# bcgsc/ntLink

Hardware: AMD Instinct MI355X
Metric: read Gbases/s mapped (ntLink pair, paf=True) (higher is better)
Workload: dtype u64

## Files before the change

include/ntlink_amd.h:

```cpp
#ifndef NTLINK_AMD_H
#define NTLINK_AMD_H

#include <stdint.h>

#ifdef __cplusplus
extern "C" {
#endif

#define NTL_OK 0
#define NTL_EINVAL (-1)
#define NTL_EDEVICE (-2)
#define NTL_ENOMEM (-3)
#define NTL_EINTERNAL (-4)
#define NTL_ERANGE (-5)
#define NTL_EIO (-6)

typedef struct ntl_ctx ntl_ctx;
typedef struct ntl_batch ntl_batch;
typedef struct ntl_sketch ntl_sketch;
typedef struct ntl_index ntl_index;
typedef struct ntl_mapres ntl_mapres;


int ntl_ctx_create(int device, ntl_ctx **out);
// ... 2 lines not shown
const char *ntl_ctx_device_name(const ntl_ctx *ctx);
int ntl_ctx_sync(ntl_ctx *ctx);
int ntl_ctx_pipelined(const ntl_ctx *ctx);
int ntl_ctx_set_pipeline(ntl_ctx *ctx, int on);
int ntl_ctx_side_stream(const ntl_ctx *ctx);

int ntl_prof_enable(ntl_ctx *ctx, int on);
int ntl_prof_reset(ntl_ctx *ctx);
int ntl_prof_get(ntl_ctx *ctx, const char *name, double *total_ms, uint64_t *launches);


int ntl_batch_create(ntl_ctx *ctx, const char *seqs, const uint64_t *offsets, uint64_t nseq,
                     ntl_batch **out);
void ntl_batch_destroy(ntl_batch *b);
uint64_t ntl_packed_words(uint64_t bases);
int ntl_batch_create_packed(ntl_ctx *ctx, const uint32_t *packed, const uint64_t *offsets, uint64_t nseq,
                            const uint32_t *seq_run_first, const uint32_t *run_start, const uint32_t *run_len, uint64_t nruns,
                            ntl_batch **out);
int ntl_batch_create_packed_at(ntl_ctx *ctx, const uint32_t *packed, uint64_t span_positions, const uint64_t *positions,
                               const uint32_t *lengths, uint64_t nseq, const uint32_t *seq_run_first, const uint32_t *run_start,
                               const uint32_t *run_len, uint64_t nruns, ntl_batch **out);
uint64_t ntl_batch_nseq(const ntl_batch *b);
uint64_t ntl_batch_bases(const ntl_batch *b);

int ntl_host_alloc(ntl_ctx *ctx, uint64_t bytes, void **out);
void ntl_host_free(ntl_ctx *ctx, void *p);


int ntl_synth_genome(ntl_ctx *ctx, uint64_t seed, const uint32_t *len, uint64_t nseq, ntl_batch **out);
int ntl_synth_slices(ntl_ctx *ctx, const ntl_batch *src, uint64_t seed, uint64_t n, const uint32_t *src_seq,
                     const uint32_t *src_start, const uint32_t *out_len, const uint8_t *reverse,
                     double sub, double ins, double del, ntl_batch **out);
int ntl_batch_download(const ntl_batch *b, char *seqs, uint64_t *offsets);


int ntl_batch_mask(ntl_ctx *ctx, const ntl_batch *src, uint64_t n, const uint32_t *src_seq, const uint32_t *keep_lo,
                   const uint32_t *keep_hi, ntl_batch **out);
int ntl_batch_download_n(const ntl_batch *b, char *seqs, uint64_t *offsets);


typedef struct ntl_ascii ntl_ascii;
typedef struct ntl_stitched ntl_stitched;
typedef struct { uint32_t store, rec, lo, hi, flags; } ntl_stitch_seg;
#define NTL_STITCH_FILL 0xFFFFFFFFu
#define NTL_STITCH_REVCOMP 1u
#define NTL_STITCH_LOWER 2u
// ... 243 lines not shown
```

ntlink_amd/capi.py:

```python
import ctypes as C
import threading
import weakref
import os

import numpy as np
from time import perf_counter as _now

_HERE = os.path.dirname(os.path.abspath(__file__))
DEFAULT_LIB = os.path.join(_HERE, "libntlink_hip.so")

SYMBOLS = [
    "ntl_ctx_create", "ntl_ctx_destroy", "ntl_last_error", "ntl_ctx_device_name", "ntl_ctx_sync", "ntl_ctx_pipelined", "ntl_ctx_set_pipeline", "ntl_ctx_side_stream",
    "ntl_prof_enable", "ntl_prof_reset", "ntl_prof_get",
    "ntl_batch_create", "ntl_batch_create_packed", "ntl_batch_create_packed_at", "ntl_packed_words", "ntl_batch_destroy", "ntl_batch_nseq", "ntl_batch_bases", "ntl_host_alloc", "ntl_host_free",
    "ntl_synth_genome", "ntl_synth_slices", "ntl_batch_download", "ntl_batch_mask", "ntl_batch_download_n",
    "ntl_ascii_create", "ntl_ascii_destroy", "ntl_ascii_nrec", "ntl_ascii_bytes", "ntl_stitch", "ntl_stitched_bytes", "ntl_stitched_copy", "ntl_stitched_destroy",
    "ntl_stitched_base_counts",
    "ntl_sketch_run", "ntl_sketch_run_indexed", "ntl_sketch_run_for_map", "ntl_sketch_has_records", "ntl_sketch_destroy", "ntl_sketch_nseq", "ntl_sketch_count", "ntl_sketch_download",
    "ntl_sketch_strips", "ntl_sketch_redo_strips", "ntl_sketch_fallback_strips", "ntl_sketch_from_lists", "ntl_sketch_plan", "ntl_sketch_wait", "ntl_mapres_wait",
    "ntl_sketch_from_host", "ntl_overlap_filter", "ntl_overlap_cuts", "ntl_path_chains",
    "ntl_index_build", "ntl_index_destroy", "ntl_index_size",
    "ntl_map_run", "ntl_mapres_destroy", "ntl_mapres_n_mappings", "ntl_mapres_n_hits", "ntl_mapres_n_pafs",
    "ntl_mapres_n_index_hits", "ntl_mapres_download", "ntl_mapres_from_host", "ntl_mapres_liftover", "ntl_map_run_grouped", "ntl_mapres_grouped_info", "ntl_mapres_gap_cuts",
    "ntl_fastx_open", "ntl_fastx_open_range", "ntl_fastx_range", "ntl_fastx_close", "ntl_fastx_error", "ntl_fastx_next", "ntl_fastx_sizes", "ntl_fastx_copy", "ntl_fastx_copy_packed", "ntl_fastx_runs", "ntl_fastx_next_span", "ntl_fastx_parse_span", "ntl_fastx_copy_span", "ntl_fastx_seqs", "ntl_fastx_offsets",
    "ntl_fastx_names", "ntl_fastx_name_offsets", "ntl_write_indexlr", "ntl_write_verbose", "ntl_write_paf",
    "ntl_tsv_open", "ntl_tsv_close", "ntl_tsv_error", "ntl_tsv_next", "ntl_tsv_sizes", "ntl_tsv_copy",
    "ntl_vmap_open", "ntl_vmap_close", "ntl_vmap_error", "ntl_vmap_next", "ntl_vmap_sizes", "ntl_vmap_copy",
    "ntl_gap_pair_table", "ntl_gap_select", "ntl_gap_cands_count", "ntl_gap_cands_copy", "ntl_gap_cands_destroy",
    "ntl_tally_create", "ntl_tally_destroy", "ntl_tally_add", "ntl_tally_npairs", "ntl_tally_ngaps", "ntl_tally_export", "ntl_tally_merge",
    "ntl_liftover",
    "ntl_names_create", "ntl_names_destroy", "ntl_mapres_format", "ntl_text_sizes", "ntl_text_download", "ntl_text_destroy", "ntl_write_blob",
    "ntl_tally_add_ends", "ntl_tally_write", "ntl_io_errno",
    "ntl_pairtab_create", "ntl_pairtab_destroy", "ntl_mapres_pairs", "ntl_pairs_count", "ntl_pairs_download", "ntl_pairs_destroy", "ntl_tally_add_pairs",
]

MAPPING_DT = np.dtype([("read", "<u4"), ("ctg", "<u4"), ("n_hits", "<u4"), ("pad", "<u4"), ("hit_off", "<u8")])
HIT_DT = np.dtype([("ctg_pos", "<u4"), ("read_pos", "<u4"), ("ctg_strand", "u1"), ("read_strand", "u1"),
# ... 74 lines not shown
    L.ntl_ctx_sync.argtypes = [vp]
    L.ntl_ctx_pipelined.argtypes = [vp]
    L.ntl_ctx_set_pipeline.argtypes = [vp, C.c_int]
    L.ntl_ctx_side_stream.argtypes = [vp]
    L.ntl_sketch_wait.argtypes = [vp]
    L.ntl_mapres_wait.argtypes = [vp]
    L.ntl_prof_enable.argtypes = [vp, C.c_int]
    L.ntl_prof_reset.argtypes = [vp]
    L.ntl_prof_get.argtypes = [vp, C.c_char_p, C.POINTER(C.c_double), u64p]
    L.ntl_batch_create.argtypes = [vp, vp, u64p, C.c_uint64, C.POINTER(vp)]
    L.ntl_batch_create_packed.argtypes = [vp, vp, u64p, C.c_uint64, vp, vp, vp, C.c_uint64, C.POINTER(vp)]
    L.ntl_batch_create_packed_at.argtypes = [vp, vp, C.c_uint64, vp, vp, C.c_uint64, vp, vp, vp, C.c_uint64, C.POINTER(vp)]
    L.ntl_fastx_next_span.argtypes = [vp, C.c_uint64, u64p, u64p]
    L.ntl_fastx_parse_span.argtypes = [vp, vp, u64p, u64p, u64p, u64p]
    L.ntl_fastx_copy_span.argtypes = [vp, vp, vp, vp, vp, vp, vp, vp, u64p]
    L.ntl_packed_words.argtypes = [C.c_uint64]
    L.ntl_packed_words.restype = C.c_uint64
    L.ntl_batch_destroy.argtypes = [vp]
    L.ntl_batch_destroy.restype = None
    L.ntl_batch_nseq.argtypes = [vp]
    L.ntl_batch_nseq.restype = C.c_uint64
    L.ntl_batch_bases.argtypes = [vp]
    L.ntl_batch_bases.restype = C.c_uint64
    L.ntl_synth_genome.argtypes = [vp, C.c_uint64, u32p, C.c_uint64, C.POINTER(vp)]
    L.ntl_synth_slices.argtypes = [vp, vp, C.c_uint64, C.c_uint64, u32p, u32p, u32p, u8p, C.c_double, C.c_double, C.c_double,
                                   C.POINTER(vp)]
    L.ntl_batch_download.argtypes = [vp, vp, u64p]
    L.ntl_batch_mask.argtypes = [vp, vp, C.c_uint64, u32p, u32p, u32p, C.POINTER(vp)]
    L.ntl_batch_download_n.argtypes = [vp, vp, u64p]
    L.ntl_ascii_create.argtypes = [vp, vp, u64p, C.c_uint64, C.POINTER(vp)]
    L.ntl_ascii_destroy.argtypes = [vp]
    L.ntl_ascii_destroy.restype = None
    for nm in ("ntl_ascii_nrec", "ntl_ascii_bytes", "ntl_stitched_bytes"):
        getattr(L, nm).argtypes = [vp]
        getattr(L, nm).restype = C.c_uint64
    L.ntl_stitch.argtypes = [vp, C.POINTER(vp), C.c_uint32, vp, C.c_uint64, C.POINTER(vp)]
    L.ntl_stitched_copy.argtypes = [vp, C.c_uint64, C.c_uint64, vp]
    L.ntl_stitched_destroy.argtypes = [vp]
    L.ntl_stitched_destroy.restype = None
    L.ntl_stitched_base_counts.argtypes = [vp, u64p, C.c_uint64, u64p]
    L.ntl_sketch_run.argtypes = [vp, vp, C.c_int, C.c_int, C.POINTER(vp)]
    L.ntl_sketch_run_indexed.argtypes = [vp, vp, C.c_int, C.c_int, vp, C.POINTER(vp)]
    L.ntl_sketch_run_for_map.argtypes = [vp, vp, C.c_int, C.c_int, vp, C.POINTER(vp)]
    L.ntl_sketch_has_records.argtypes = [vp]
    L.ntl_sketch_destroy.argtypes = [vp]
    L.ntl_sketch_destroy.restype = None
# ... 137 lines not shown
        try:
            self.close()
        except Exception:
            pass

    def __enter__(self):
        return self

    def __exit__(self, *a):
        self.close()


class Batch(_Handle):
    _destroy = "ntl_batch_destroy"

    @property
    def nseq(self):
        return int(self.dev.L.ntl_batch_nseq(self.ptr))

    @property
    def bases(self):
        return int(self.dev.L.ntl_batch_bases(self.ptr))

    def download(self):
        buf = np.empty(max(self.bases, 1), np.uint8)
        off = np.zeros(self.nseq + 1, np.uint64)
        self.dev._chk(self.dev.L.ntl_batch_download(self.ptr, buf.ctypes.data, _ptr(off, C.c_uint64)))
        return buf[:self.bases], off

    def download_n(self):
        off = np.zeros(self.nseq + 1, np.uint64)
        buf = np.empty(max(self.bases, 1), np.uint8)
        self.dev._chk(self.dev.L.ntl_batch_download_n(self.ptr, buf.ctypes.data, _ptr(off, C.c_uint64)))
        return buf[:int(off[-1])], off


class Ascii(_Handle):
    _destroy = "ntl_ascii_destroy"

    @property
    def nrec(self):
        return int(self.dev.L.ntl_ascii_nrec(self.ptr))

    @property
    def nbytes(self):
        return int(self.dev.L.ntl_ascii_bytes(self.ptr))
# ... 537 lines not shown
```

ntlink_amd/csrc/ntl_hip.hip:

```cpp
#include <hip/hip_runtime.h>
#include <stdint.h>
#include <stdio.h>
#include <stdlib.h>
#include <string.h>
#include <algorithm>
#include <atomic>
#include <chrono>
#include <deque>
#include <map>
#include <unordered_map>
#include <mutex>
#include <memory>
#include <string>
#include <thread>
#include <vector>

#include "../../include/ntlink_amd.h"
#include "dev_common.h"
#include "dev_pool.h"
#include "pending.h"
#include "scan_kernels.h"
#include "sketch_kernels.h"
#include "sketch2_kernels.h"
#include "sketch_small_kernels.h"
// ... 424 lines not shown
    return NTL_OK;
}


static int device_scan(ntl_ctx *c, const uint32_t *in, uint32_t *out, uint64_t n, uint32_t *total_host, unsigned batch = 1,
                       uint32_t *sums_dev = nullptr, int sid = SID_MAIN)
{
    const uint64_t tiles = scan_tile_count(n);
    DevBuf tile;
    int rc;
    hipStream_t st = c->s(sid);
    if ((rc = tile.alloc(c, tiles * 4 * batch, sid))) return rc;
    scan_launch(st, in, out, n, batch, tile.as<uint32_t>(), sums_dev);
    HIPCHK(c, hipGetLastError());
    if (total_host) {
        for (unsigned y = 0; y < batch; y++)
            HIPCHK(c, hipMemcpyAsync(total_host + y, out + y * (n + 1) + n, 4, hipMemcpyDeviceToHost, st));
        HIPCHK(c, hipStreamSynchronize(st));
    }
    return NTL_OK;
}


struct ntl_batch {
    ntl_ctx *c;
    std::atomic<int> refs{1};
    uint64_t nseq = 0, bases = 0, nruns = 0, total_gpos = 0, nwords_packed = 0;
    bool any_multi = false;
    DevBuf packed, seq_base, seq_run_first, run_start, run_len;
    DevBuf seq_len_dev;
    const uint32_t *d_seq_len = nullptr;
    std::vector<uint32_t> seq_len;
    hipEvent_t ready = nullptr;
    mutable bool w_waited = false;
};

static void batch_unref(const ntl_batch *cb)
{
    ntl_batch *b = const_cast<ntl_batch *>(cb);
    if (b && --b->refs == 0) {
        (void)hipSetDevice(b->c->device);
        b->c->pq.event_put(b->ready);
        delete b;
    }
}

static void batch_on_wstream(ntl_ctx *c, const ntl_batch *b)
{
    if (!c->pipelined) return;
    if (b->ready && !b->w_waited) { (void)hipStreamWaitEvent(c->wstream, b->ready, 0); b->w_waited = true; }
    for (int sid : {(int)SID_W, (int)SID_S}) {
        b->packed.touch(sid); b->seq_base.touch(sid); b->seq_run_first.touch(sid); b->run_start.touch(sid); b->run_len.touch(sid);
    }
}

static std::unique_ptr<ntl_batch> batch_new(ntl_ctx *c, uint64_t nseq, uint64_t bases, uint64_t span)
{
    std::unique_ptr<ntl_batch> b(new ntl_batch());
    b->c = c; b->nseq = nseq; b->bases = bases;
    b->total_gpos = NTL_LEAD_PAD + span;
    b->nwords_packed = (NTL_LEAD_PAD + span + NTL_END_PAD + 15) / 16 + 2;
    return b;
}

// ... 875 lines not shown
    if (G.LW < 2 && C != 16) {
        C = 16;
        G.a = (w - C) / C; G.r0 = (w - C) % C;
        nt = SK_NT;
        G.LW = nt - (G.a + 2);
    }
    G.NWO = G.LW * C - 1;
    if (G.LW < 2 || G.NWO < 1) {
        char msg[160];
        snprintf(msg, sizeof msg, "window size w=%d is beyond this build's limit of w <= %d (a strip of %d x 16 k-mers must hold two windows' lanes)",
                 w, NTL_MAX_W, SK_NT);
        return fail(c, NTL_EINVAL, msg);
    }
    return NTL_OK;
}

static int window_plan(ntl_ctx *c, const ntl_batch *b, int k, int w, bool no_lists, WindowPlan &P)
{
    memset(&P, 0, sizeof P);
    bool small;
    int rc;
    if ((rc = sketch_geometry(c, k, w, P.G, P.C, P.nt, small))) return rc;
    const SketchGeom &G = P.G;
    auto count_strips = [&]() {
        P.strips = 0;
        for (uint64_t i = 0; i < b->nseq; i++) {
            const uint64_t len = b->seq_len[i];
            if (len + 2 > (uint64_t)k + (uint64_t)w) P.strips += (len - k - w + 2 + (uint64_t)G.NWO - 1) / (uint64_t)G.NWO;
        }
    };
    count_strips();
    if (P.strips >= 0x7FFFFFFFull) return fail(c, NTL_EINVAL, "batch too large: too many strips");
    bool fast = P.C == 16 && k <= 16 * SK2_QMAX && G.a + 2 <= SK2_PAD && !small;
    if (const char *e = getenv("NTL_SKETCH_FAST")) fast = fast && atoi(e) != 0;
    P.pass = small ? WP_SMALL : WP_EXACT_ONLY;
    if (!fast) return NTL_OK;
    const char *te = getenv("NTL_SKETCH_THRESH");
    double cpw = te ? atof(te) : 10.0;
    if (cpw == 1.0) cpw = 10.0;
    if (cpw > 0 && P.nt != 128 && 4096.0 * cpw / w <= WP_FIT_THRESH) P.thresh = (uint32_t)std::min(4294967295.0, 4294967296.0 * cpw / w);
    if (const char *e = getenv("NTL_SKETCH_ABLATE")) P.dbg = atoi(e);
    if (const char *e = getenv("NTL_SKETCH_FORCE_REDO")) P.force_redo = atoi(e);
    P.expected_per_strip = 4096.0 * (double)P.thresh / 4294967296.0;
    P.dense_windows = P.expected_per_strip > WP_FIT_15_6;
    const bool sparse = P.thresh && (P.dbg & ~24) == 0;
    const char *we = getenv("NTL_SKETCH_WAVE");
// ... 93 lines not shown
    return true;
}

static void launch_give_up_pass(hipStream_t st, const WindowPlan &P, const Sketch2Args &B)
{
    const unsigned strips = B.A.nstrips;
    with_constant<0, 16>(P.G.r0, [&](auto r0) {
        constexpr int R0 = decltype(r0)::value;
        const dim3 lgrid(std::min(strips, 4096u));
        if (P.nt == SK_NT_LONG && P.big) hipLaunchKernelGGL((sketch_fast_list_kernel<SK_NT_LONG, R0, true>), lgrid, dim3(SK_NT_LONG), 0, st, B, (const uint32_t *)B.fb_list, (const uint32_t *)B.fb_count);
        else if (P.nt == SK_NT_LONG) hipLaunchKernelGGL((sketch_fast_list_kernel<SK_NT_LONG, R0>), lgrid, dim3(SK_NT_LONG), 0, st, B, (const uint32_t *)B.fb_list, (const uint32_t *)B.fb_count);
        else if (P.big) hipLaunchKernelGGL((sketch_fast_list_kernel<256, R0, true>), lgrid, dim3(256), 0, st, B, (const uint32_t *)B.fb_list, (const uint32_t *)B.fb_count);
        else hipLaunchKernelGGL((sketch_fast_list_kernel<256, R0>), lgrid, dim3(256), 0, st, B, (const uint32_t *)B.fb_list, (const uint32_t *)B.fb_count);
    });
}

struct SketchWork {
    int wsid; hipStream_t ws, ms;
    int ssid; hipStream_t ss;
    int psid; hipStream_t ps;
    hipStream_t last;
    static int order(ntl_ctx *c, hipStream_t on, hipStream_t then);
    uint64_t nmask;
    DevBuf run_n, run_ord, seq_M, nstrips, strip_first, tile, redo, strip_tab;
    SeqTables T; StripLists Ls = {}; StripZero Z = {};
    DevBuf lcnt, lent, loff;
    struct Mask : CleanMask {
        ntl_ctx *c = nullptr;
        ~Mask() { if (p) c->mem.free_uncached(p, bytes); }
    } mask;
    DevBuf strip_lite;
};
static const uint64_t REDO_HEAD = 16 + 8 * 16;

int SketchWork::order(ntl_ctx *c, hipStream_t on, hipStream_t then)
{
    if (on == then) return NTL_OK;
    hipEvent_t e = c->pq.event_get();
    if (!e) return fail(c, NTL_EDEVICE, "hipEventCreate failed");
    HIPCHK(c, hipEventRecord(e, on));
    HIPCHK(c, hipStreamWaitEvent(then, e, 0));
    c->pq.event_put(e);
    return NTL_OK;
}

static int sketch_prepare(ntl_ctx *c, const ntl_batch *b, int k, int w, const WindowPlan &P, ntl_sketch *s, SketchWork &W)
{
    const uint64_t nseq = b->nseq, ub_strips = P.strips;
    const int wsid = W.wsid, psid = W.psid;
    auto window_stage_uses = [&](const DevBuf &d) { d.touch(wsid); d.touch(W.ssid); };
    int rc;
    W.nmask = (b->total_gpos + 31) / 32 + 1;
    if ((rc = W.run_n.alloc(c, (b->nruns + 1) * 4, psid)) || (rc = W.run_ord.alloc(c, (b->nruns + 1) * 4, psid)) ||
        (rc = W.seq_M.alloc(c, (nseq + 1) * 4, psid)) || (rc = W.nstrips.alloc(c, (nseq + 1) * 4, psid)) ||
        (rc = W.strip_first.alloc(c, (nseq + 2) * 4, psid)) || (rc = s->mx_off.alloc(c, (nseq + 1) * 4)) ||
        (rc = s->sums.alloc(c, sizeof(SketchSums), psid))) return rc;
    window_stage_uses(W.run_n); window_stage_uses(W.run_ord); window_stage_uses(W.seq_M);
    s->sums.touch(SID_MAIN);
    batch_on_wstream(c, b);
    if (W.ps != W.ws && b->ready) HIPCHK(c, hipStreamWaitEvent(W.ps, b->ready, 0));
    SeqTables &T = W.T;
    T.packed = b->packed.as<uint32_t>(); T.seq_base = b->seq_base.as<uint64_t>();
    T.seq_run_first = b->seq_run_first.as<uint32_t>(); T.run_start = b->run_start.as<uint32_t>();
    T.run_len = b->run_len.as<uint32_t>(); T.nseq = (uint32_t)nseq;
    StripLists &Ls = W.Ls;
    if (P.lists) {
        Ls.slot = P.slot; Ls.ovf_base = (uint32_t)((ub_strips + 1) * P.slot); Ls.ovf_cap = P.pool;
        if ((rc = W.lcnt.alloc(c, (ub_strips + 4) * 4, psid)) || (rc = W.lent.alloc(c, ((ub_strips + 1) * P.slot + P.pool) * 4, wsid)) || (rc = W.loff.alloc(c, (ub_strips + 2) * 4))) return rc;
        window_stage_uses(W.lcnt); window_stage_uses(W.lent);
        W.lcnt.touch(SID_MAIN); W.lent.touch(SID_MAIN);
        Ls.cnt = W.lcnt.as<uint32_t>(); Ls.ent = W.lent.as<uint32_t>(); Ls.ctl = Ls.cnt + ub_strips + 2;
    }
    StripZero &Z = W.Z;
    if (P.fast() && ub_strips) {
        if ((rc = W.redo.alloc(c, (REDO_HEAD + 2 * ub_strips + 4) * 4, psid))) return rc;
        window_stage_uses(W.redo);
        Z.head = W.redo.as<uint32_t>(); Z.nhead = (uint32_t)REDO_HEAD;
        Z.cnt = Ls.cnt; Z.ncnt = Ls.cnt ? (uint32_t)(ub_strips + 4) : 0u;
    }
    W.mask.c = c;
    if (!P.lists && (rc = mask_take(c, W.nmask * 4, wsid, &W.mask))) return rc;
    if ((rc = W.strip_tab.alloc(c, (ub_strips + 1) * sizeof(StripInfo), psid)) || (rc = W.strip_lite.alloc(c, (ub_strips + 1) * sizeof(StripLite), psid))) return rc;
    window_stage_uses(W.strip_tab); window_stage_uses(W.strip_lite);
    SketchSums *dsums = s->sums.as<SketchSums>();
    Z.sums = (uint32_t *)dsums; Z.nsums = (uint32_t)(sizeof(SketchSums) / 4);
    if (!nseq) HIPCHK(c, hipMemsetAsync(dsums, 0, sizeof(SketchSums), W.ms));
    ProfSpan sp(c, "sketch_meta", psid);
    if (nseq) {
        KTables K;
        K.run_n = W.run_n.as<uint32_t>(); K.run_ord = W.run_ord.as<uint32_t>();
        K.seq_M = W.seq_M.as<uint32_t>(); K.seq_nstrips = W.nstrips.as<uint32_t>();
        hipLaunchKernelGGL(seq_meta_kernel, dim3((unsigned)((nseq + 255) / 256)), dim3(256), 0, W.ps, T, K, k, w, P.G.NWO);
        HIPCHK(c, hipGetLastError());
        if ((rc = device_scan(c, W.nstrips.as<uint32_t>(), W.strip_first.as<uint32_t>(), nseq, nullptr, 1, nullptr, psid))) return rc;
        hipLaunchKernelGGL(strip_table_kernel, dim3((unsigned)((ub_strips + 255) / 256 + 1)), dim3(256), 0, W.ps, T, (const uint32_t *)K.run_n,
                           (const uint32_t *)K.run_ord, (const uint32_t *)K.seq_M, (const uint32_t *)W.strip_first.as<uint32_t>(), P.G.NWO,
                           P.C * P.nt, W.strip_tab.as<StripInfo>(), (uint32_t)ub_strips + 1u, W.strip_lite.as<StripLite>(), Z);
        HIPCHK(c, hipGetLastError());
    }
    return NTL_OK;
}

static int g8k_for(ntl_ctx *c, int k, hipStream_t ws, uint32_t rev_a, uint32_t rev_b, const uint2 **out)
{
    auto it = c->g8k.find(k);
    if (it == c->g8k.end()) {
        if (c->g8k.size() >= 8) {
            HIPCHK(c, sync_both(c));
            for (auto &kv : c->g8k) (void)hipFree(kv.second);
            c->g8k.clear();
        }
        void *t = nullptr;
        if (hipMalloc(&t, (size_t)(2 * 65536 + 1024) * sizeof(uint2)) != hipSuccess) return fail(c, NTL_ENOMEM, "hipMalloc failed");
        hipLaunchKernelGGL(g8k_build_kernel, dim3(256), dim3(256), 0, ws, (const uint64_t (*)[2])c->g8, (uint2 *)t, rev_a, rev_b);
        hipLaunchKernelGGL(g4k_build_kernel, dim3(1), dim3(256), 0, ws, (const uint64_t (*)[2])c->g4, (uint2 *)t + 2 * 65536, rev_a, rev_b);
        HIPCHK(c, hipGetLastError());
        it = c->g8k.emplace(k, t).first;
    }
    *out = (const uint2 *)it->second;
    return NTL_OK;
}

static int sketch_window_stage(ntl_ctx *c, const ntl_batch *b, int k, const WindowPlan &P, ntl_sketch *s, SketchWork &W)
{
    const uint64_t ub_strips = P.strips;
    int rc;
    W.last = W.ws;
    if ((rc = SketchWork::order(c, W.ps, W.ws))) return rc;
    if (!ub_strips) return NTL_OK;
    const int wsid = W.wsid, nt = P.nt;
    SketchArgs A = {};
    A.T = W.T;
    A.run_n = W.run_n.as<uint32_t>(); A.run_ord = W.run_ord.as<uint32_t>(); A.seq_M = W.seq_M.as<uint32_t>();
    A.strip_lite = W.strip_lite.as<StripLite>(); A.strip_tab = W.strip_tab.as<StripInfo>(); A.nstrips = (uint32_t)ub_strips; A.mask = (uint32_t *)W.mask.p; A.G = P.G;
    make_tables(k, A.roll_tab, A.seed_tab);
    A.g4 = (const uint64_t (*)[2])c->g4; A.g8 = (const uint64_t (*)[2])c->g8;
    A.Ls = W.Ls;
    if (!P.fast()) {
        ProfSpan sp(c, "sketch_mask", wsid);
        if (P.pass == WP_SMALL) launch_small(c, A, (unsigned)ub_strips, b->any_multi);
        else if (P.C == 16) launch_mask<16>(W.ws, A, (unsigned)ub_strips, true, b->any_multi, nt);
        else if (P.C == 4) launch_mask<4>(W.ws, A, (unsigned)ub_strips, true, b->any_multi, nt);
        else launch_mask<1>(W.ws, A, (unsigned)ub_strips, true, b->any_multi, nt);
        HIPCHK(c, hipGetLastError());
        return NTL_OK;
    }
    uint32_t *const redo = W.redo.as<uint32_t>();
    Sketch2Args B = {};
    B.A = A;
    B.thresh = P.thresh; B.dbg = P.dbg; B.force_redo = P.force_redo;
    B.redo_count = redo; B.fb_count = redo + 1; B.chunk_next = redo + 16;
    B.redo_list = redo + REDO_HEAD; B.fb_list = B.redo_list + ub_strips + 2;
    B.max_word = b->nwords_packed - 1;
    B.q16 = k / 16; B.r16 = k % 16; B.rev_a = (uint32_t)(k - 1) % 33u; B.rev_b = (uint32_t)(k - 1) % 31u;
    if ((rc = g8k_for(c, k, W.ws, B.rev_a, B.rev_b, &B.g8k))) return rc;
    B.g4k = B.g8k + 2 * 65536;
    bool gave_up;
// ... 45 lines not shown
    else if (probe == 0 && (eu ? emit_u >= 4 : small)) hipLaunchKernelGGL((emit_kernel<0, 4, NTL_EMIT_DENSE_CAP>), g, dim3(EMIT_NT), 0, ms, E);
    else if (probe == 0 && emit_u >= 2) hipLaunchKernelGGL((emit_kernel<0, 2>), g, dim3(EMIT_NT), 0, ms, E);
    else if (probe == 0) hipLaunchKernelGGL((emit_kernel<0, 1>), g, dim3(EMIT_NT), 0, ms, E);
    else with_constant<1, 3>(probe, [&](auto p) {
        constexpr int PROBE = decltype(p)::value;
        if (emit_u >= 2) hipLaunchKernelGGL((emit_kernel<PROBE, 2>), g, dim3(EMIT_NT), 0, ms, E);
        else hipLaunchKernelGGL((emit_kernel<PROBE, 1>), g, dim3(EMIT_NT), 0, ms, E);
    });
}

static int sketch_emit_stage(ntl_ctx *c, const ntl_batch *b, int k, const WindowPlan &P, const ntl_index *ix, ntl_sketch *s, uint64_t cap, SketchWork &W)
{
    const bool lists = P.lists;
    const uint64_t nseq = b->nseq, ub_strips = P.strips, nmask = W.nmask;
    hipStream_t ms = W.ms;
    const StripLists &Ls = W.Ls;
    SketchSums *dsums = s->sums.as<SketchSums>();
    int rc;
    ProfSpan sp(c, "sketch_emit");
    const uint64_t tiles = lists ? (ub_strips + EL_STRIPS - 1) / EL_STRIPS : (nmask + EMIT_TILE - 1) / EMIT_TILE;
    DevBuf tile_seq, tile_next;
    if ((rc = tile_next.alloc(c, 8 * 16 * 4))) return rc;
    if (lists) {
        W.strip_first.touch(SID_MAIN); W.strip_tab.touch(SID_MAIN);
        if ((rc = device_scan(c, Ls.cnt, W.loff.as<uint32_t>(), ub_strips, nullptr, 1, &dsums->total_mx))) return rc;
        SketchSums *hd = (SketchSums *)c->pq.slot_dev(s->lz.slot);
        hipLaunchKernelGGL(list_fail_kernel, dim3(1), dim3(64), 0, ms, (const uint32_t *)Ls.ctl, &dsums->total_mx, &dsums->list_fail, tile_next.as<uint32_t>(),
                           &hd->total_mx, &hd->list_fail);
        hipLaunchKernelGGL(mx_off_from_strips_kernel, dim3((unsigned)((nseq + 256) / 256)), dim3(256), 0, ms, (const uint32_t *)W.strip_first.as<uint32_t>(),
                           (const uint32_t *)W.loff.as<uint32_t>(), (uint32_t)nseq, s->mx_off.as<uint32_t>());
    } else {
        if ((rc = W.tile.alloc(c, tiles * 4)) || (rc = tile_seq.alloc(c, (tiles + 2) * 4))) return rc;
        if (nseq)
            hipLaunchKernelGGL(tile_seq_kernel, dim3((unsigned)((nseq + 255) / 256)), dim3(256), 0, ms, (const uint64_t *)W.T.seq_base, (uint32_t)nseq, tiles, tile_seq.as<uint32_t>());
        hipLaunchKernelGGL(mask_count_kernel, dim3((unsigned)tiles), dim3(EMIT_NT), 0, ms, (const uint32_t *)W.mask.p, nmask, W.tile.as<uint32_t>(), tile_next.as<uint32_t>());
        hipLaunchKernelGGL(scan_tiles_kernel, dim3(1), dim3(SCAN_NT), 0, ms, W.tile.as<uint32_t>(), tiles, &dsums->total_mx, (uint64_t)0, (uint32_t *)nullptr);
    }
    HIPCHK(c, hipGetLastError());
    if (!s->no_records && (rc = s->records.alloc(c, cap * sizeof(MxRecord)))) return rc;
    s->cap = cap;
    const int probe = !ix ? 0 : (ix->hit_fraction->load(std::memory_order_relaxed) <= 0.5f ? 1 : 2);
    if (ix) {
        if ((rc = s->rpos.alloc(c, cap * 4)) || (rc = s->cand.alloc(c, cap * sizeof(Cand)))) return rc;
        s->cand_gen = ix->gen;
        if (ix->c != c && ix->built) HIPCHK(c, hipStreamWaitEvent(ms, ix->built, 0));
    }
    EmitArgs E = {};
    E.packed = W.T.packed; E.seq_base = W.T.seq_base; E.nseq = (uint32_t)nseq; E.mask = (uint32_t *)W.mask.p;
    E.nwords = nmask; E.tile_off = W.tile.as<uint32_t>(); E.tile_seq = tile_seq.as<uint32_t>(); E.mx_off = s->mx_off.as<uint32_t>();
    E.out = s->no_records ? nullptr : s->records.as<MxRecord>(); E.out_cap = (uint32_t)cap;
    E.k = k; E.mult = 1ull ^ ((uint64_t)k * 0x90b45d39fb6da1faull);
    uint64_t roll[16][2];
    make_tables(k, roll, E.seed_tab);
    E.g4 = (const uint64_t (*)[2])c->g4; E.g8 = (const uint64_t (*)[2])c->g8;
    if (ix) {
        E.rpos = s->rpos.as<uint32_t>();
        E.slots = ix->slots.as<IndexSlot>(); E.tags = ix->tags.as<uint8_t>(); E.special = ix->special.as<IndexSpecial>();
        E.ix_bits = ix->bits; E.cand = s->cand.as<Cand>(); E.nfound = &dsums->nfound;
    }
    const EmitGrid eg = emit_grid(c->pipelined, probe, lists, P.dense_windows, c->n_cu, tiles);
    E.ntiles = (uint32_t)tiles; E.tile_next = eg.from_counters ? tile_next.as<uint32_t>() : nullptr;
    EmitListArgs Q = {};
    if (lists) { Q.Ls = Ls; Q.strip_tab = W.strip_tab.as<StripInfo>(); Q.strip_off = W.loff.as<uint32_t>(); Q.nstrips = (uint32_t)ub_strips; }
    emit_launch(ms, eg.grid, lists, probe, P.pass == WP_SMALL, E, Q);
    HIPCHK(c, hipGetLastError());
    if (W.mask.p) {
        CleanMask m = W.mask;
        m.clean = c->pq.event_get();
        if (m.clean) HIPCHK(c, hipEventRecord(m.clean, ms));
        else HIPCHK(c, hipStreamSynchronize(ms));
        c->masks.push_back(m);
        W.mask.p = nullptr;
    }
    s->nfound_owed = false;
    if (!lists) {
        SketchSums *hs = (SketchSums *)s->lz.slot;
        HIPCHK(c, hipMemcpyAsync(&hs->total_mx, &dsums->total_mx, 4, hipMemcpyDeviceToHost, ms));
        if (ix) HIPCHK(c, hipMemcpyAsync(&hs->nfound, &dsums->nfound, 8, hipMemcpyDeviceToHost, ms));
    } else s->nfound_owed = ix != nullptr;
    return NTL_OK;
}

static int sketch_enqueue(ntl_ctx *c, const ntl_batch *b, int k, int w, const ntl_index *ix, ntl_sketch *s, uint64_t cap)
{
    hipEvent_t &throttle = c->throttle[c->n_enqueued & 7u];
    if (throttle) (void)hipEventSynchronize(throttle);
// ... 63 lines not shown
            s->nfound_owed = false;
            hipLaunchKernelGGL(sketch_nfound_kernel, dim3(1), dim3(64), 0, c->stream, (const unsigned long long *)&s->sums.as<SketchSums>()->nfound,
                               &((SketchSums *)c->pq.slot_dev(lz.slot))->nfound);
            hipError_t le = hipGetLastError();
            if (le == hipSuccess) le = hipEventRecord(lz.done, c->stream);
            if (le != hipSuccess) { pending_abort(c, lz, fail(c, NTL_EDEVICE, std::string("sketch: ") + hipGetErrorString(le))); break; }
        }
        const hipError_t e = lz.wait();
        lz.pending = false;
        if (e != hipSuccess) { lz.failed = fail(c, NTL_EDEVICE, std::string("sketch: ") + hipGetErrorString(e)); break; }
        const SketchSums hs = *(const SketchSums *)lz.slot;
        s->count = hs.total_mx; s->redo_strips = hs.redo_n; s->fallback_strips = hs.fb_n; s->nfound = hs.nfound;
        if (s->count <= s->cap && !hs.list_fail) break;
        if (round || !s->src) { lz.failed = fail(c, NTL_EINTERNAL, "sketch: the exact-size round overflowed again"); break; }
        if (hs.list_fail) s->no_lists = true;
        s->gen++;
        memset(lz.slot, 0, sizeof(PinSlot));
        const int rc = sketch_enqueue(c, s->src, s->k, s->w, (const ntl_index *)lz.holds[0].p, s, s->count);
        if (rc) { pending_abort(c, lz, rc); break; }
    }
    if (s->src) { batch_unref(s->src); s->src = nullptr; }
    lz.settle(c->pq);
    return lz.failed;
}

extern "C" int ntl_sketch_run(ntl_ctx *c, const ntl_batch *b, int k, int w, ntl_sketch **out)
{
    return sketch_run_impl(c, b, k, w, nullptr, out);
}

extern "C" int ntl_sketch_run_indexed(ntl_ctx *c, const ntl_batch *b, int k, int w, const ntl_index *ix, ntl_sketch **out)
{
    if (!ix) return NTL_EINVAL;
    if (ix->c->device != c->device) return fail(c, NTL_EINVAL, "the index lives on another device");
    return sketch_run_impl(c, b, k, w, ix, out);
}

extern "C" int ntl_sketch_run_for_map(ntl_ctx *c, const ntl_batch *b, int k, int w, const ntl_index *ix, ntl_sketch **out)
{
    if (!ix) return NTL_EINVAL;
    if (ix->c->device != c->device) return fail(c, NTL_EINVAL, "the index lives on another device");
    return sketch_run_impl(c, b, k, w, ix, out, true);
}

extern "C" int ntl_sketch_has_records(const ntl_sketch *s) { return s && !s->no_records; }

// ... 1284 lines not shown
```

ntlink_amd/csrc/sketch_kernels.h:

```cpp
#pragma once
#include "dev_common.h"
#include "index_common.h"

struct SeqTables {
    const uint32_t *packed;
    const uint64_t *seq_base;
    const uint32_t *seq_run_first;
    const uint32_t *run_start;
    const uint32_t *run_len;
    uint32_t nseq;
};

struct KTables {
    uint32_t *run_n;
    uint32_t *run_ord;
    uint32_t *seq_M;
    uint32_t *seq_nstrips;
};

struct SketchGeom {
    int k, w;
    int a;
    int r0;
    int LW;
// ... 62 lines not shown
    if ((drop >> 5) == (uint32_t)L) m &= ~(1u << (drop & 31u));
    uint32_t total;
    uint32_t at = block_excl_scan<NT>((uint32_t)__popc(m), s_tmp, total);
    if (L == 0) s_tmp[0] = strip_list_place(Ls, strip, total);
    __syncthreads();
    const uint32_t first = s_tmp[0];
    if (first != NTL_NONE) {
        uint32_t *const dst = Ls.ent + first;
        while (m) {
            const uint32_t b = (uint32_t)__ffs(m) - 1u;
            m &= m - 1u;
            dst[at++] = pos_of(32u * (uint32_t)L + b);
        }
    }
    __syncthreads();
}

struct StripZero {
    uint32_t *cnt; uint32_t ncnt;
    uint32_t *head; uint32_t nhead;
    uint32_t *sums; uint32_t nsums;
};

__global__ void strip_table_kernel(SeqTables T, const uint32_t *run_n, const uint32_t *run_ord, const uint32_t *seq_M,
                                   const uint32_t *strip_first, int NWO, int strip_elems, StripInfo *tab, uint32_t cap, StripLite *lite,
                                   StripZero Z)
{
    const uint32_t i = blockIdx.x * blockDim.x + threadIdx.x;
    for (uint32_t j = i; j < Z.ncnt; j += gridDim.x * blockDim.x) Z.cnt[j] = 0u;
    if (i < Z.nhead) Z.head[i] = 0u;
    if (i < Z.nsums) Z.sums[i] = 0u;
    if (i >= cap) return;
    if (i >= strip_first[T.nseq]) {
        tab[i].seq = NTL_NONE;
        if (lite) { lite[i].g0 = 0; lite[i].hi = 0; lite[i].p0 = 0; }
        return;
    }
    uint32_t lo = 0, hi = T.nseq;
    while (hi - lo > 1) {
        const uint32_t mid = (lo + hi) >> 1;
        if (strip_first[mid] <= i) lo = mid; else hi = mid;
    }
    const uint32_t s = lo;
    StripInfo I;
    I.seq = s;
    I.E0 = (int32_t)((i - strip_first[s]) * (uint32_t)NWO) - 1;
    I.M = seq_M[s];
    I.base = T.seq_base[s];
    const uint32_t e_lo = I.E0 < 0 ? 0u : (uint32_t)I.E0;
    uint32_t e_hi = (uint32_t)(I.E0 + strip_elems);
    if (e_hi > I.M) e_hi = I.M;
    const uint32_t g0 = T.seq_run_first[s], g1 = T.seq_run_first[s + 1];
    uint32_t rl = g0, rh = g1;
    while (rh - rl > 1) {
// ... 673 lines not shown
```

ntlink_amd/csrc/window_plan.h:

```cpp
#pragma once
#include "sketch2_kernels.h"

static const double WP_FIT_THRESH = 580.0;
static const double WP_FIT_WAVE = 440.0;
static const double WP_FIT_STAGED = 340.0;
static const double WP_FIT_15_6 = 300.0;
static const double WP_FIT_11_4 = 175.0;

enum WindowPass { WP_SMALL, WP_EXACT_ONLY,  WP_BLOCK_MINIMA, WP_THRESH, WP_WAVE };
enum WaveShape { WS_8_11_4, WS_8_15_6, WS_8_19_8, WS_4_19_8, WS_8_19_7_L128, WS_DEFAULTS, WS_4_11_4 = WS_DEFAULTS, WS_16_11_4 };

struct WindowPlan {
    SketchGeom G;
    int C, nt;
    uint64_t strips;
    WindowPass pass;
    bool big, direct;
    WaveShape shape;
    unsigned beside;
    int wgs_per_cu;
    uint32_t chunk_budget;
    uint32_t thresh;
    int dbg, force_redo;
    double expected_per_strip;
    bool dense_windows;
    bool lists;
    uint32_t slot, pool;
    bool fast() const { return pass >= WP_BLOCK_MINIMA; }
};

#define NTL_WAVE_SHAPES(X) \
    X(WS_8_11_4, 8, 11, 4, 64) X(WS_8_15_6, 8, 15, 6, 64) X(WS_8_19_8, 8, 19, 8, 64) X(WS_4_19_8, 4, 19, 8, 64) \
    X(WS_8_19_7_L128, 8, 19, 7, 128) X(WS_4_11_4, 4, 11, 4, 64) X(WS_16_11_4, 16, 11, 4, 64)

template <typename F>
static void with_wave_kernel(WaveShape shape, F &&f)
{
    switch (shape) {
#define NTL_WAVE_CASE(id, waves, slots, rounds, cl) case id: return f(sketch_wave_kernel<waves, slots, rounds, cl>, 64u * waves);
    NTL_WAVE_SHAPES(NTL_WAVE_CASE)
#undef NTL_WAVE_CASE
    }
}

static void wave_shape_numbers(WaveShape shape, int32_t out[4])
{
    switch (shape) {
#define NTL_WAVE_CASE(id, waves, slots, rounds, cl) case id: out[0] = waves; out[1] = slots; out[2] = rounds; out[3] = cl; return;
    NTL_WAVE_SHAPES(NTL_WAVE_CASE)
#undef NTL_WAVE_CASE
// ... 3 lines not shown
```

ntlink_amd/pipeline.py:

```python
import datetime
import json
import os
import sys
import time

import numpy as np

from . import capi, formats, pairing, seqio

TSV_BLOCK_BYTES = 256 << 20
DEFAULT_BATCH_BASES = 512_000_000


_TRACE = [] if os.environ.get("NTL_PIPE_TRACE") else None


def _mark(what, seq=-1):
    if _TRACE is not None:
        import threading
        _TRACE.append((time.perf_counter(), threading.current_thread().name, what, seq))


def _log(*a):
    print(datetime.datetime.today(), ":", *a, file=sys.stdout, flush=True)
# ... 477 lines not shown
                    return None
                rs_ = next(it, None)
                if rs_ is None:
                    return None
                if len(rs_):
                    seq = state["next_seq"]
                    state["next_seq"] += 1
                    now = time.perf_counter()
                    stats["t_ingest"] += max(0.0, now - state["t_mark"])
                    state["t_mark"] = now
                    return seq, rs_

    def work(wdev):
        try:
            while True:
                got = take()
                if got is None:
                    return
                seq, rs_ = got
                _mark("dev_start", seq)
                t_dev = time.perf_counter()
                rl = rs_.lengths
                with (wdev.batch_packed(rs_) if rs_.packed is not None else wdev.batch(rs_.buf, rs_.offsets)) as rb:
                    t_up = time.perf_counter()
                    dev.pinned_release(rs_.pinned if rs_.packed is not None else rs_.buf)
                    rs_.buf = rs_.packed = rs_.pinned = None
                    with wdev.sketch(rb, map_kw["k"], w, index=ix, records=False) as rsk:
                        t_sk = time.perf_counter()
                        with wdev.map(ix, rsk, rl, **map_kw) as res:
                            t_mp = time.perf_counter()
                            pres = None if records else {}
                            if records and text is not None:
                                try:
                                    with wdev.names(rs_.names, rl) as rn, res.format(rn, text[0], text[1], text[2]) as txt:
                                        pres = txt.download()
                                except capi.NtlError as exc:
                                    if getattr(exc, "code", 0) != capi.NTL_ERANGE:
                                        raise
                            if pres is None:
                                pres = res.download(pinned=True)
                            if pairs is not None:
                                pres["pairs"] = wdev.mapres_pairs(res, pairs, rl)
                            n_mx, n_hit = rsk.count, res.n_index_hits
                t_done = time.perf_counter()
                _mark("dev_done", seq)
                parts = (t_up - t_dev, t_sk - t_up, t_mp - t_sk, t_done - t_mp)
# ... 190 lines not shown
```

Measured before the change: 1649.

## Cache per-batch strip geometry tables and build them at batch upload

Moves the strip metadata build (seq_meta kernel, scan, strip table) into a reference-counted StripGeom cached on the batch, keyed by k, w and the plan geometry. Repeated sketches of the same batch can then reuse it. The pipeline builds it right after upload via a new ntl_batch_prepare call. The zeroing of list counters is split into its own small kernel. The cache adds cross-stream event waits and lifetime bookkeeping. In the pair pipeline each batch is sketched once, so the main effect is moving work earlier, not removing it.

```diff
diff --git a/include/ntlink_amd.h b/include/ntlink_amd.h
--- a/include/ntlink_amd.h
+++ b/include/ntlink_amd.h
@@ -48,6 +48,7 @@
                                const uint32_t *run_len, uint64_t nruns, ntl_batch **out);
 uint64_t ntl_batch_nseq(const ntl_batch *b);
 uint64_t ntl_batch_bases(const ntl_batch *b);
+int ntl_batch_prepare(ntl_ctx *ctx, const ntl_batch *b, int k, int w);
 
 int ntl_host_alloc(ntl_ctx *ctx, uint64_t bytes, void **out);
 void ntl_host_free(ntl_ctx *ctx, void *p);
diff --git a/ntlink_amd/capi.py b/ntlink_amd/capi.py
--- a/ntlink_amd/capi.py
+++ b/ntlink_amd/capi.py
@@ -12,7 +12,7 @@
 SYMBOLS = [
     "ntl_ctx_create", "ntl_ctx_destroy", "ntl_last_error", "ntl_ctx_device_name", "ntl_ctx_sync", "ntl_ctx_pipelined", "ntl_ctx_set_pipeline", "ntl_ctx_side_stream",
     "ntl_prof_enable", "ntl_prof_reset", "ntl_prof_get",
-    "ntl_batch_create", "ntl_batch_create_packed", "ntl_batch_create_packed_at", "ntl_packed_words", "ntl_batch_destroy", "ntl_batch_nseq", "ntl_batch_bases", "ntl_host_alloc", "ntl_host_free",
+    "ntl_batch_create", "ntl_batch_create_packed", "ntl_batch_create_packed_at", "ntl_packed_words", "ntl_batch_destroy", "ntl_batch_nseq", "ntl_batch_bases", "ntl_batch_prepare", "ntl_host_alloc", "ntl_host_free",
     "ntl_synth_genome", "ntl_synth_slices", "ntl_batch_download", "ntl_batch_mask", "ntl_batch_download_n",
     "ntl_ascii_create", "ntl_ascii_destroy", "ntl_ascii_nrec", "ntl_ascii_bytes", "ntl_stitch", "ntl_stitched_bytes", "ntl_stitched_copy", "ntl_stitched_destroy",
     "ntl_stitched_base_counts",
@@ -133,6 +133,8 @@
     L.ntl_batch_nseq.restype = C.c_uint64
     L.ntl_batch_bases.argtypes = [vp]
     L.ntl_batch_bases.restype = C.c_uint64
+    L.ntl_batch_prepare.argtypes = [vp, vp, C.c_int, C.c_int]
+    L.ntl_batch_prepare.restype = C.c_int
     L.ntl_synth_genome.argtypes = [vp, C.c_uint64, u32p, C.c_uint64, C.POINTER(vp)]
     L.ntl_synth_slices.argtypes = [vp, vp, C.c_uint64, C.c_uint64, u32p, u32p, u32p, u8p, C.c_double, C.c_double, C.c_double,
                                    C.POINTER(vp)]
@@ -316,6 +318,10 @@
     def bases(self):
         return int(self.dev.L.ntl_batch_bases(self.ptr))
 
+    def prepare(self, k, w, dev=None):
+        dev = dev or self.dev
+        dev._chk(dev.L.ntl_batch_prepare(dev.ptr, self.ptr, int(k), int(w)))
+
     def download(self):
         buf = np.empty(max(self.bases, 1), np.uint8)
         off = np.zeros(self.nseq + 1, np.uint64)
diff --git a/ntlink_amd/csrc/ntl_hip.hip b/ntlink_amd/csrc/ntl_hip.hip
--- a/ntlink_amd/csrc/ntl_hip.hip
+++ b/ntlink_amd/csrc/ntl_hip.hip
@@ -470,6 +470,33 @@
 }
 
 
+struct StripGeom {
+    ntl_ctx *c = nullptr;
+    std::atomic<int> refs{1};
+    bool shared = false;
+    int k = 0, w = 0, NWO = 0, strip_elems = 0;
+    uint64_t ub_strips = 0;
+    DevBuf run_n, run_ord, seq_M, nstrips, strip_first, strip_tab, strip_lite;
+    hipEvent_t built = nullptr;
+    hipStream_t built_on = nullptr;
+    bool is(int k_, int w_, int NWO_, int elems_, uint64_t ub_) const { return k == k_ && w == w_ && NWO == NWO_ && strip_elems == elems_ && ub_strips == ub_; }
+    uint64_t bytes() const { return run_n.bytes + run_ord.bytes + seq_M.bytes + nstrips.bytes + strip_first.bytes + strip_tab.bytes + strip_lite.bytes; }
+};
+
+static void geom_unref(const StripGeom *cg)
+{
+    StripGeom *g = const_cast<StripGeom *>(cg);
+    if (!g || --g->refs != 0) return;
+    (void)hipSetDevice(g->c->device);
+    for (DevBuf *d : {&g->run_n, &g->run_ord, &g->seq_M, &g->nstrips, &g->strip_first, &g->strip_tab, &g->strip_lite}) {
+        if (d->p) g->c->mem.free_uncached(d->p, d->bytes);
+        d->p = nullptr;
+    }
+    if (g->built) (void)hipEventDestroy(g->built);
+    delete g;
+}
+static void hold_geom(const void *g, void *) { geom_unref((const StripGeom *)g); }
+
 struct ntl_batch {
     ntl_ctx *c;
     std::atomic<int> refs{1};
@@ -481,6 +508,8 @@
     std::vector<uint32_t> seq_len;
     hipEvent_t ready = nullptr;
     mutable bool w_waited = false;
+    mutable std::mutex geo_mu;
+    mutable StripGeom *geo = nullptr;
 };
 
 static void batch_unref(const ntl_batch *cb)
@@ -488,6 +517,7 @@
     ntl_batch *b = const_cast<ntl_batch *>(cb);
     if (b && --b->refs == 0) {
         (void)hipSetDevice(b->c->device);
+        geom_unref(b->geo);
         b->c->pq.event_put(b->ready);
         delete b;
     }
@@ -1409,6 +1439,8 @@
     int rc;
     if ((rc = sketch_geometry(c, k, w, P.G, P.C, P.nt, small))) return rc;
     const SketchGeom &G = P.G;
+    P.strip_cache = true;
+    if (const char *e = getenv("NTL_STRIP_CACHE")) P.strip_cache = atoi(e) != 0;
     auto count_strips = [&]() {
         P.strips = 0;
         for (uint64_t i = 0; i < b->nseq; i++) {
@@ -1548,14 +1580,15 @@
     hipStream_t last;
     static int order(ntl_ctx *c, hipStream_t on, hipStream_t then);
     uint64_t nmask;
-    DevBuf run_n, run_ord, seq_M, nstrips, strip_first, tile, redo, strip_tab;
+    DevBuf tile, redo;
+    StripGeom own;
+    const StripGeom *geo = nullptr;
     SeqTables T; StripLists Ls = {}; StripZero Z = {};
     DevBuf lcnt, lent, loff;
     struct Mask : CleanMask {
         ntl_ctx *c = nullptr;
         ~Mask() { if (p) c->mem.free_uncached(p, bytes); }
     } mask;
-    DevBuf strip_lite;
 };
 static const uint64_t REDO_HEAD = 16 + 8 * 16;
 
@@ -1570,6 +1603,73 @@
     return NTL_OK;
 }
 
+static SeqTables batch_tables(const ntl_batch *b)
+{
+    SeqTables T;
+    T.packed = b->packed.as<uint32_t>(); T.seq_base = b->seq_base.as<uint64_t>();
+    T.seq_run_first = b->seq_run_first.as<uint32_t>(); T.run_start = b->run_start.as<uint32_t>();
+    T.run_len = b->run_len.as<uint32_t>(); T.nseq = (uint32_t)b->nseq;
+    return T;
+}
+
+static int geometry_build(ntl_ctx *c, const ntl_batch *b, int k, int w, const WindowPlan &P, int sid, StripGeom &G)
+{
+    const uint64_t nseq = b->nseq, ub_strips = P.strips;
+    int rc;
+    sid = c->sid(sid);
+    G.c = c; G.k = k; G.w = w; G.NWO = P.G.NWO; G.strip_elems = P.C * P.nt; G.ub_strips = ub_strips;
+    G.built_on = c->s(sid);
+    if ((rc = G.run_n.alloc(c, (b->nruns + 1) * 4, sid)) || (rc = G.run_ord.alloc(c, (b->nruns + 1) * 4, sid)) ||
+        (rc = G.seq_M.alloc(c, (nseq + 1) * 4, sid)) || (rc = G.nstrips.alloc(c, (nseq + 1) * 4, sid)) ||
+        (rc = G.strip_first.alloc(c, (nseq + 2) * 4, sid)) || (rc = G.strip_tab.alloc(c, (ub_strips + 1) * sizeof(StripInfo), sid)) ||
+        (rc = G.strip_lite.alloc(c, (ub_strips + 1) * sizeof(StripLite), sid))) return rc;
+    if (!nseq) return NTL_OK;
+    ProfSpan sp(c, "sketch_meta", sid);
+    hipStream_t st = G.built_on;
+    const SeqTables T = batch_tables(b);
+    KTables K;
+    K.run_n = G.run_n.as<uint32_t>(); K.run_ord = G.run_ord.as<uint32_t>();
+    K.seq_M = G.seq_M.as<uint32_t>(); K.seq_nstrips = G.nstrips.as<uint32_t>();
+    hipLaunchKernelGGL(seq_meta_kernel, dim3((unsigned)((nseq + 255) / 256)), dim3(256), 0, st, T, K, k, w, P.G.NWO);
+    HIPCHK(c, hipGetLastError());
+    if ((rc = device_scan(c, G.nstrips.as<uint32_t>(), G.strip_first.as<uint32_t>(), nseq, nullptr, 1, nullptr, sid))) return rc;
+    hipLaunchKernelGGL(strip_table_kernel, dim3((unsigned)((ub_strips + 255) / 256 + 1)), dim3(256), 0, st, T, (const uint32_t *)K.run_n,
+                       (const uint32_t *)K.run_ord, (const uint32_t *)K.seq_M, (const uint32_t *)G.strip_first.as<uint32_t>(), P.G.NWO,
+                       P.C * P.nt, G.strip_tab.as<StripInfo>(), (uint32_t)ub_strips + 1u, G.strip_lite.as<StripLite>());
+    HIPCHK(c, hipGetLastError());
+    if (G.shared) {
+        HIPCHK(c, hipEventCreateWithFlags(&G.built, hipEventDisableTiming));
+        HIPCHK(c, hipEventRecord(G.built, st));
+    }
+    return NTL_OK;
+}
+
+static int geometry_get(ntl_ctx *c, const ntl_batch *b, int k, int w, const WindowPlan &P, int sid, const StripGeom **out)
+{
+    *out = nullptr;
+    if (!P.strip_cache) return NTL_OK;
+    std::lock_guard<std::mutex> lock(b->geo_mu);
+    if (b->geo && b->geo->is(k, w, P.G.NWO, P.C * P.nt, P.strips)) {
+        b->geo->refs++;
+        *out = b->geo;
+        return NTL_OK;
+    }
+    if (c != b->c) return NTL_OK;
+    StripGeom *g = new StripGeom();
+    g->shared = true;
+    if (int rc = geometry_build(c, b, k, w, P, sid, *g)) {
+        (void)sync_both(c);
+        geom_unref(g);
+        return rc;
+    }
+    StripGeom *old = b->geo;
+    b->geo = g;
+    g->refs++;
+    geom_unref(old);
+    *out = g;
+    return NTL_OK;
+}
+
 static int sketch_prepare(ntl_ctx *c, const ntl_batch *b, int k, int w, const WindowPlan &P, ntl_sketch *s, SketchWork &W)
 {
     const uint64_t nseq = b->nseq, ub_strips = P.strips;
@@ -1577,18 +1677,28 @@
     auto window_stage_uses = [&](const DevBuf &d) { d.touch(wsid); d.touch(W.ssid); };
     int rc;
     W.nmask = (b->total_gpos + 31) / 32 + 1;
-    if ((rc = W.run_n.alloc(c, (b->nruns + 1) * 4, psid)) || (rc = W.run_ord.alloc(c, (b->nruns + 1) * 4, psid)) ||
-        (rc = W.seq_M.alloc(c, (nseq + 1) * 4, psid)) || (rc = W.nstrips.alloc(c, (nseq + 1) * 4, psid)) ||
-        (rc = W.strip_first.alloc(c, (nseq + 2) * 4, psid)) || (rc = s->mx_off.alloc(c, (nseq + 1) * 4)) ||
-        (rc = s->sums.alloc(c, sizeof(SketchSums), psid))) return rc;
-    window_stage_uses(W.run_n); window_stage_uses(W.run_ord); window_stage_uses(W.seq_M);
+    if ((rc = s->mx_off.alloc(c, (nseq + 1) * 4)) || (rc = s->sums.alloc(c, sizeof(SketchSums), psid))) return rc;
     s->sums.touch(SID_MAIN);
     batch_on_wstream(c, b);
     if (W.ps != W.ws && b->ready) HIPCHK(c, hipStreamWaitEvent(W.ps, b->ready, 0));
-    SeqTables &T = W.T;
-    T.packed = b->packed.as<uint32_t>(); T.seq_base = b->seq_base.as<uint64_t>();
-    T.seq_run_first = b->seq_run_first.as<uint32_t>(); T.run_start = b->run_start.as<uint32_t>();
-    T.run_len = b->run_len.as<uint32_t>(); T.nseq = (uint32_t)nseq;
+    const StripGeom *shared = nullptr;
+    if ((rc = geometry_get(c, b, k, w, P, psid, &shared))) return rc;
+    if (shared) {
+        Hold &h = s->lz.holds[1];
+        if (h.p) h.release(h.p, c);
+        h = {shared, hold_geom};
+        W.geo = shared;
+        if (shared->built && shared->built_on != W.ps && hipEventQuery(shared->built) != hipSuccess) {
+            (void)hipGetLastError();
+            HIPCHK(c, hipStreamWaitEvent(W.ps, shared->built, 0));
+        }
+    } else {
+        if ((rc = geometry_build(c, b, k, w, P, psid, W.own))) return rc;
+        window_stage_uses(W.own.run_n); window_stage_uses(W.own.run_ord); window_stage_uses(W.own.seq_M);
+        window_stage_uses(W.own.strip_tab); window_stage_uses(W.own.strip_lite);
+        W.geo = &W.own;
+    }
+    W.T = batch_tables(b);
     StripLists &Ls = W.Ls;
     if (P.lists) {
         Ls.slot = P.slot; Ls.ovf_base = (uint32_t)((ub_strips + 1) * P.slot); Ls.ovf_cap = P.pool;
@@ -1606,22 +1716,12 @@
     }
     W.mask.c = c;
     if (!P.lists && (rc = mask_take(c, W.nmask * 4, wsid, &W.mask))) return rc;
-    if ((rc = W.strip_tab.alloc(c, (ub_strips + 1) * sizeof(StripInfo), psid)) || (rc = W.strip_lite.alloc(c, (ub_strips + 1) * sizeof(StripLite), psid))) return rc;
-    window_stage_uses(W.strip_tab); window_stage_uses(W.strip_lite);
     SketchSums *dsums = s->sums.as<SketchSums>();
     Z.sums = (uint32_t *)dsums; Z.nsums = (uint32_t)(sizeof(SketchSums) / 4);
     if (!nseq) HIPCHK(c, hipMemsetAsync(dsums, 0, sizeof(SketchSums), W.ms));
-    ProfSpan sp(c, "sketch_meta", psid);
     if (nseq) {
-        KTables K;
-        K.run_n = W.run_n.as<uint32_t>(); K.run_ord = W.run_ord.as<uint32_t>();
-        K.seq_M = W.seq_M.as<uint32_t>(); K.seq_nstrips = W.nstrips.as<uint32_t>();
-        hipLaunchKernelGGL(seq_meta_kernel, dim3((unsigned)((nseq + 255) / 256)), dim3(256), 0, W.ps, T, K, k, w, P.G.NWO);
-        HIPCHK(c, hipGetLastError());
-        if ((rc = device_scan(c, W.nstrips.as<uint32_t>(), W.strip_first.as<uint32_t>(), nseq, nullptr, 1, nullptr, psid))) return rc;
-        hipLaunchKernelGGL(strip_table_kernel, dim3((unsigned)((ub_strips + 255) / 256 + 1)), dim3(256), 0, W.ps, T, (const uint32_t *)K.run_n,
-                           (const uint32_t *)K.run_ord, (const uint32_t *)K.seq_M, (const uint32_t *)W.strip_first.as<uint32_t>(), P.G.NWO,
-                           P.C * P.nt, W.strip_tab.as<StripInfo>(), (uint32_t)ub_strips + 1u, W.strip_lite.as<StripLite>(), Z);
+        ProfSpan sp(c, "sketch_zero", psid);
+        hipLaunchKernelGGL(strip_zero_kernel, dim3((unsigned)std::min<uint64_t>((ub_strips + 255) / 256 + 1, 1024)), dim3(256), 0, W.ps, Z);
         HIPCHK(c, hipGetLastError());
     }
     return NTL_OK;
@@ -1657,8 +1757,8 @@
     const int wsid = W.wsid, nt = P.nt;
     SketchArgs A = {};
     A.T = W.T;
-    A.run_n = W.run_n.as<uint32_t>(); A.run_ord = W.run_ord.as<uint32_t>(); A.seq_M = W.seq_M.as<uint32_t>();
-    A.strip_lite = W.strip_lite.as<StripLite>(); A.strip_tab = W.strip_tab.as<StripInfo>(); A.nstrips = (uint32_t)ub_strips; A.mask = (uint32_t *)W.mask.p; A.G = P.G;
+    A.run_n = W.geo->run_n.as<uint32_t>(); A.run_ord = W.geo->run_ord.as<uint32_t>(); A.seq_M = W.geo->seq_M.as<uint32_t>();
+    A.strip_lite = W.geo->strip_lite.as<StripLite>(); A.strip_tab = W.geo->strip_tab.as<StripInfo>(); A.nstrips = (uint32_t)ub_strips; A.mask = (uint32_t *)W.mask.p; A.G = P.G;
     make_tables(k, A.roll_tab, A.seed_tab);
     A.g4 = (const uint64_t (*)[2])c->g4; A.g8 = (const uint64_t (*)[2])c->g8;
     A.Ls = W.Ls;
@@ -1750,12 +1850,12 @@
     DevBuf tile_seq, tile_next;
     if ((rc = tile_next.alloc(c, 8 * 16 * 4))) return rc;
     if (lists) {
-        W.strip_first.touch(SID_MAIN); W.strip_tab.touch(SID_MAIN);
+        if (W.geo == &W.own) { W.own.strip_first.touch(SID_MAIN); W.own.strip_tab.touch(SID_MAIN); }
         if ((rc = device_scan(c, Ls.cnt, W.loff.as<uint32_t>(), ub_strips, nullptr, 1, &dsums->total_mx))) return rc;
         SketchSums *hd = (SketchSums *)c->pq.slot_dev(s->lz.slot);
         hipLaunchKernelGGL(list_fail_kernel, dim3(1), dim3(64), 0, ms, (const uint32_t *)Ls.ctl, &dsums->total_mx, &dsums->list_fail, tile_next.as<uint32_t>(),
                            &hd->total_mx, &hd->list_fail);
-        hipLaunchKernelGGL(mx_off_from_strips_kernel, dim3((unsigned)((nseq + 256) / 256)), dim3(256), 0, ms, (const uint32_t *)W.strip_first.as<uint32_t>(),
+        hipLaunchKernelGGL(mx_off_from_strips_kernel, dim3((unsigned)((nseq + 256) / 256)), dim3(256), 0, ms, (const uint32_t *)W.geo->strip_first.as<uint32_t>(),
                            (const uint32_t *)W.loff.as<uint32_t>(), (uint32_t)nseq, s->mx_off.as<uint32_t>());
     } else {
         if ((rc = W.tile.alloc(c, tiles * 4)) || (rc = tile_seq.alloc(c, (tiles + 2) * 4))) return rc;
@@ -1789,7 +1889,7 @@
     const EmitGrid eg = emit_grid(c->pipelined, probe, lists, P.dense_windows, c->n_cu, tiles);
     E.ntiles = (uint32_t)tiles; E.tile_next = eg.from_counters ? tile_next.as<uint32_t>() : nullptr;
     EmitListArgs Q = {};
-    if (lists) { Q.Ls = Ls; Q.strip_tab = W.strip_tab.as<StripInfo>(); Q.strip_off = W.loff.as<uint32_t>(); Q.nstrips = (uint32_t)ub_strips; }
+    if (lists) { Q.Ls = Ls; Q.strip_tab = W.geo->strip_tab.as<StripInfo>(); Q.strip_off = W.loff.as<uint32_t>(); Q.nstrips = (uint32_t)ub_strips; }
     emit_launch(ms, eg.grid, lists, probe, P.pass == WP_SMALL, E, Q);
     HIPCHK(c, hipGetLastError());
     if (W.mask.p) {
@@ -1899,6 +1999,19 @@
     if (s->src) { batch_unref(s->src); s->src = nullptr; }
     lz.settle(c->pq);
     return lz.failed;
+}
+
+extern "C" int ntl_batch_prepare(ntl_ctx *c, const ntl_batch *b, int k, int w)
+{
+    if (!c || !b) return NTL_EINVAL;
+    (void)hipSetDevice(c->device);
+    WindowPlan P;
+    if (int rc = window_plan(c, b, k, w, false, P)) return rc;
+    if (c != b->c) return NTL_OK;
+    const StripGeom *g = nullptr;
+    if (int rc = geometry_get(c, b, k, w, P, SID_MAIN, &g)) return rc;
+    geom_unref(g);
+    return NTL_OK;
 }
 
 extern "C" int ntl_sketch_run(ntl_ctx *c, const ntl_batch *b, int k, int w, ntl_sketch **out)
diff --git a/ntlink_amd/csrc/sketch_kernels.h b/ntlink_amd/csrc/sketch_kernels.h
--- a/ntlink_amd/csrc/sketch_kernels.h
+++ b/ntlink_amd/csrc/sketch_kernels.h
@@ -108,14 +108,18 @@
     uint32_t *sums; uint32_t nsums;
 };
 
-__global__ void strip_table_kernel(SeqTables T, const uint32_t *run_n, const uint32_t *run_ord, const uint32_t *seq_M,
-                                   const uint32_t *strip_first, int NWO, int strip_elems, StripInfo *tab, uint32_t cap, StripLite *lite,
-                                   StripZero Z)
+__global__ void strip_zero_kernel(StripZero Z)
 {
     const uint32_t i = blockIdx.x * blockDim.x + threadIdx.x;
     for (uint32_t j = i; j < Z.ncnt; j += gridDim.x * blockDim.x) Z.cnt[j] = 0u;
     if (i < Z.nhead) Z.head[i] = 0u;
     if (i < Z.nsums) Z.sums[i] = 0u;
+}
+
+__global__ void strip_table_kernel(SeqTables T, const uint32_t *run_n, const uint32_t *run_ord, const uint32_t *seq_M,
+                                   const uint32_t *strip_first, int NWO, int strip_elems, StripInfo *tab, uint32_t cap, StripLite *lite)
+{
+    const uint32_t i = blockIdx.x * blockDim.x + threadIdx.x;
     if (i >= cap) return;
     if (i >= strip_first[T.nseq]) {
         tab[i].seq = NTL_NONE;
diff --git a/ntlink_amd/csrc/window_plan.h b/ntlink_amd/csrc/window_plan.h
--- a/ntlink_amd/csrc/window_plan.h
+++ b/ntlink_amd/csrc/window_plan.h
@@ -26,6 +26,7 @@
     bool dense_windows;
     bool lists;
     uint32_t slot, pool;
+    bool strip_cache;
     bool fast() const { return pass >= WP_BLOCK_MINIMA; }
 };
 
diff --git a/ntlink_amd/pipeline.py b/ntlink_amd/pipeline.py
--- a/ntlink_amd/pipeline.py
+++ b/ntlink_amd/pipeline.py
@@ -523,6 +523,7 @@
                 t_dev = time.perf_counter()
                 rl = rs_.lengths
                 with (wdev.batch_packed(rs_) if rs_.packed is not None else wdev.batch(rs_.buf, rs_.offsets)) as rb:
+                    rb.prepare(map_kw["k"], w)
                     t_up = time.perf_counter()
                     dev.pinned_release(rs_.pinned if rs_.packed is not None else rs_.buf)
                     rs_.buf = rs_.packed = rs_.pinned = None
```

Result: no change. 1635 (-0.8%).
